# quinlan-lab/STRling

Measured on AMD Instinct MI355X. Metric: reads/sec through extract+cluster, 30x 150 bp WGS; 1/2/4/8 MI355X + CPU ref, higher is better.
Workload: dtype u8/u32 integer; 1 GPU; 1xMI355X: 30x 150 bp PE synthetic WGS, k=2-6 repeat-unit scorer + soft-clip scan + device pair logic + on-GPU radix-sort/segmented clustering (BASELINE.json configs[1]+[2]); reads_per_gpu=33554432, read_len=150, unique_reads_per_gpu=33554432, tiles=1, scored_reads=2843008, soft_items=993737, str_reads_clustered=514295, clusters=322142, bounds=5047, parallelism=records sharded over 1 GPU(s), no data-path collective

## Files before the change

### strling_amd/csrc/device_util.h

```cpp
#pragma once
#include <algorithm>
#include "common.h"

namespace strl {

__device__ __forceinline__ void bloom_set(uint32_t *bloom, uint32_t mask, uint64_t m) {
  const uint32_t b0 = (uint32_t)m & mask, b1 = (uint32_t)(m >> 32) & mask;
  atomicOr(&bloom[b0 >> 5], 1u << (b0 & 31u));
  atomicOr(&bloom[b1 >> 5], 1u << (b1 & 31u));
}
__device__ __forceinline__ bool bloom_test(const uint32_t *bloom, uint32_t mask, uint64_t m) {
  const uint32_t b0 = (uint32_t)m & mask;
  if (!((bloom[b0 >> 5] >> (b0 & 31u)) & 1u)) return false;
  const uint32_t b1 = (uint32_t)(m >> 32) & mask;
  return (bloom[b1 >> 5] >> (b1 & 31u)) & 1u;
}


static __global__ void zero_words_kernel(uint32_t *p, size_t n_words) {
  const size_t n4 = n_words / 4, stride = (size_t)gridDim.x * blockDim.x;
  uint4 *q = reinterpret_cast<uint4 *>(p);
  for (size_t i = (size_t)blockIdx.x * blockDim.x + threadIdx.x; i < n4; i += stride) q[i] = make_uint4(0, 0, 0, 0);
  if (blockIdx.x == 0 && threadIdx.x < (n_words & 3)) p[n4 * 4 + threadIdx.x] = 0;
}
static __global__ void zero_words2_kernel(uint32_t *p, size_t n_words, uint32_t *q, size_t m_words) {
  const size_t stride = (size_t)gridDim.x * blockDim.x, i0 = (size_t)blockIdx.x * blockDim.x + threadIdx.x;
  for (size_t i = i0; i < n_words; i += stride) p[i] = 0;
  for (size_t i = i0; i < m_words; i += stride) q[i] = 0;
}
static inline hipError_t zero_words2(void *p, size_t bytes, void *q, size_t qbytes, hipStream_t st) {
  const size_t w = std::max(bytes, qbytes) / 4;
  if (!w) return hipSuccess;
  const unsigned blocks = (unsigned)std::min<size_t>((w + 255) / 256, 1024);
  hipLaunchKernelGGL(zero_words2_kernel, dim3(blocks), dim3(256), 0, st, static_cast<uint32_t *>(p), bytes / 4, static_cast<uint32_t *>(q), qbytes / 4);
  return hipGetLastError();
}
static inline hipError_t zero_words(void *p, size_t bytes, hipStream_t st) {
  const size_t words = bytes / 4;
  if (!words) return hipSuccess;
  const unsigned blocks = (unsigned)std::min<size_t>((words / 4 + 255) / 256 + 1, 1024);
  hipLaunchKernelGGL(zero_words_kernel, dim3(blocks), dim3(256), 0, st, static_cast<uint32_t *>(p), words);
  return hipGetLastError();
}
}
```

### strling_amd/csrc/pair.hip

```cpp
#include <string.h>
#include <algorithm>
#include "common.h"
#include "device_util.h"
#include "sort.h"
#include "front.h"

namespace strl {

constexpr uint16_t F_PROPER = 0x2, F_REVERSE = 0x10, F_MREVERSE = 0x20, F_SECONDARY = 0x100, F_SUPPL = 0x800;
constexpr int PAIR_MAXM = 15;
constexpr int PAIR_LONG_MAX = PAIR_LONG_MAX_ITEMS;
constexpr uint32_t PAIR_SPILL_CAP = 1u << 16;

struct PairParams {
  uint32_t n;
  uint32_t tail_start;
  const strl_pair_rec *rec;
  const uint64_t *qhash;
  const uint32_t *whole;
  const strl_soft_rec *soft;
  const uint32_t *d_n_soft;
  uint32_t scap;
  uint32_t *bloom;
  uint32_t bloom_mask;
  uint64_t *item_key;
  uint32_t *item_val;
  uint32_t item_cap;
  uint32_t *pc;
  strl_tread *emit;
  uint64_t *emit_key;
  uint32_t *emit_val;
  uint32_t emit_cap;
  double p;
  uint32_t min_mapq;
  int32_t frag_median;
  uint32_t *spill;
  const uint64_t *qref;
  const uint8_t *qarena;
};

__device__ inline bool qname_differs(const PairParams &P, uint32_t r0, uint32_t r1) {
  if (!P.qref) return false;
  const uint64_t a = P.qref[r0], b = P.qref[r1];
  if ((a & 255u) != (b & 255u)) return true;
  const uint8_t *x = P.qarena + (a >> 8), *y = P.qarena + (b >> 8);
  for (uint32_t j = 0; j < (uint32_t)(a & 255u); ++j) if (x[j] != y[j]) return true;
  return false;
}

__global__ __launch_bounds__(1024) void pair_soft_items_kernel(PairParams P) {
  __shared__ uint32_t wcnt[128];
  __shared__ uint32_t base_sh;
  constexpr int U = 2;
  const int lane = threadIdx.x & 63, wave = threadIdx.x >> 6;
  const unsigned long long below = (1ull << lane) - 1ull;
  uint32_t n_src = *P.d_n_soft;
  if (n_src > P.scap) n_src = P.scap;
  for (uint32_t b0 = blockIdx.x * (1024u * U); b0 < n_src; b0 += gridDim.x * (1024u * U)) {
    uint64_t m[U];
    bool hot[U];
    unsigned long long bal[U];
#pragma unroll
    for (int u = 0; u < U; ++u) {
      const uint32_t j = b0 + 1024u * u + threadIdx.x;
      hot[u] = false;
      m[u] = 0;
      if (j < n_src) {
        const strl_soft_rec s = P.soft[j];
        hot[u] = (STRL_RES_COUNT(s.res_first) | STRL_RES_COUNT(s.res_after)) != 0;
        if (hot[u]) {
          m[u] = fmix64(P.qhash[s.read_side >> 1]);
          bloom_set(P.bloom, P.bloom_mask, m[u]);
        }
      }
    }
#pragma unroll
    for (int u = 0; u < U; ++u) {
      bal[u] = __ballot(hot[u]);
      if (lane == 0) wcnt[u * 16 + wave] = (uint32_t)__popcll(bal[u]);
    }
    __syncthreads();
    if (threadIdx.x == 0) {
      uint32_t tot = 0;
      for (int w = 0; w < 16 * U; ++w) { const uint32_t c = wcnt[w]; wcnt[w] = tot; tot += c; }
      base_sh = tot ? atomicAdd(&P.pc[PC_ITEMS], tot) : 0u;
    }
    __syncthreads();
#pragma unroll
    for (int u = 0; u < U; ++u) {
      if (hot[u]) {
        const uint32_t d = base_sh + wcnt[u * 16 + wave] + (uint32_t)__popcll(bal[u] & below);
        if (d < P.item_cap) { P.item_key[d] = m[u]; P.item_val[d] = 0x80000000u | (b0 + 1024u * u + threadIdx.x); }
        else atomicOr(&P.pc[PC_ERR], PAIR_ERR_ITEMS);
      }
    }
    __syncthreads();
  }
}

constexpr int PR_STAGE = 1024, PR_ILP = 8;
__global__ __launch_bounds__(256) void pair_probe_kernel(PairParams P) {
  __shared__ uint32_t stage[4][PR_STAGE + 64 * PR_ILP];
  const int lane = threadIdx.x & 63, wave = threadIdx.x >> 6;
  uint32_t *buf = stage[wave];
  const uint64_t n_waves = (uint64_t)gridDim.x * 4u;
  const uint64_t gw = (uint64_t)blockIdx.x * 4u + wave;
  const uint64_t per = (((P.n + n_waves - 1) / n_waves) + 63ull) & ~63ull;
  const uint64_t r0 = gw * per;
  const uint64_t r1 = r0 + per < P.n ? r0 + per : P.n;
  const unsigned long long below = (1ull << lane) - 1ull;
  uint32_t cnt = 0;
  auto flush = [&]() {
    if (cnt) {
      uint32_t b = 0;
      if (lane == 0) b = atomicAdd(&P.pc[PC_ITEMS], cnt);
      b = __shfl(b, 0);
      __builtin_amdgcn_wave_barrier();
      for (uint32_t i = lane; i < cnt; i += 64) {
        const uint32_t r = buf[i];
        const uint32_t d = b + i;
        if (d < P.item_cap) { P.item_key[d] = fmix64(P.qhash[r]); P.item_val[d] = r; }
        else atomicOr(&P.pc[PC_ERR], PAIR_ERR_ITEMS);
      }
      __builtin_amdgcn_wave_barrier();
      cnt = 0;
    }
  };
  uint64_t cur[PR_ILP], nxt[PR_ILP];
  auto load = [&](uint64_t base, uint64_t (&x)[PR_ILP]) {
#pragma unroll
    for (int j = 0; j < PR_ILP; ++j) {
      const uint64_t r = base + 64ull * j + lane;
      x[j] = r < r1 ? P.qhash[r] : 0ull;
    }
  };
  load(r0, cur);
  for (uint64_t base = r0; base < r1; base += 64 * PR_ILP) {
    load(base + 64 * PR_ILP, nxt);
    uint64_t m[PR_ILP];
    uint32_t w0[PR_ILP];
#pragma unroll
    for (int j = 0; j < PR_ILP; ++j) {
      m[j] = fmix64(cur[j]);
      w0[j] = P.bloom[((uint32_t)m[j] & P.bloom_mask) >> 5];
    }
    bool hit[PR_ILP];
#pragma unroll
    for (int j = 0; j < PR_ILP; ++j) {
      const uint64_t r = base + 64ull * j + lane;
      hit[j] = r < r1 && ((w0[j] >> ((uint32_t)m[j] & 31u)) & 1u);
    }
#pragma unroll
    for (int j = 0; j < PR_ILP; ++j) {
      if (hit[j]) {
        const uint32_t b1 = (uint32_t)(m[j] >> 32) & P.bloom_mask;
        hit[j] = (P.bloom[b1 >> 5] >> (b1 & 31u)) & 1u;
      }
    }
#pragma unroll
    for (int j = 0; j < PR_ILP; ++j) {
      const unsigned long long mk = __ballot(hit[j]);
      if (hit[j]) buf[cnt + __popcll(mk & below)] = (uint32_t)(base + 64ull * j + lane);
      cnt += (uint32_t)__popcll(mk);
    }
    if (cnt >= PR_STAGE) flush();
#pragma unroll
    for (int j = 0; j < PR_ILP; ++j) cur[j] = nxt[j];
  }
  flush();
}

struct DTread {
  int32_t tid;
  uint32_t position;
  uint32_t k, code;
  uint16_t flag;
  uint8_t split, mapq, count, align_length;
  uint32_t qid;
};

__device__ __forceinline__ double p_repeat(const DTread &t) {
  const uint8_t prod = (uint8_t)(t.count * (uint8_t)t.k);
  const uint8_t al = t.align_length ? t.align_length : 1;
  return (double)prod / (double)al;
}
__device__ inline uint32_t min_rev_complement(uint32_t code, uint32_t k) {
  if (k == 0) return code;
  uint32_t c = 0;
  for (int i = (int)k - 1; i >= 0; --i) c = (c << 2) | (3u - ((code >> (2 * (k - 1 - i))) & 3u));
  const uint32_t mask = (1u << (2 * k)) - 1u;
  uint32_t best = c, f = c;
  for (uint32_t j = 0; j < k; ++j) {
    f = ((f << 2) | (f >> (2 * (k - 1)))) & mask;
    best = f < best ? f : best;
  }
  return best;
}
__device__ inline uint32_t canonical_repeat(uint32_t code, uint32_t k) {
  const uint32_t r = min_rev_complement(code, k);
  for (uint32_t j = 0; j < k; ++j) {
    const uint32_t a = (r >> (2 * (k - 1 - j))) & 3u, b = (code >> (2 * (k - 1 - j))) & 3u;
    const uint32_t ra = a ^ 1u, rb = b ^ 1u;
    if (ra != rb) return ra < rb ? r : code;
  }
  return code;
}
__device__ __forceinline__ bool should_reverse(uint16_t f) {
  const bool r = !(f & F_MREVERSE);
  return (f & F_REVERSE) ? !r : r;
}
__device__ inline bool adjust_by(DTread &A, const DTread &B, const PairParams &P, uint32_t B_position) {
  if (A.count == 0) return false;
  const uint32_t half = (uint32_t)((double)A.align_length / 2.0 + 0.5);
  if (B.mapq > P.min_mapq && ((p_repeat(A) > P.p && p_repeat(B) < 0.2) || (!(A.flag & F_PROPER) && A.mapq < P.min_mapq))) {
    if (B.flag & F_REVERSE) {
// ... 152 lines not shown
      mate.code = canonical_repeat(mate.code, mate.k);
      mate.position = 0;
      mate.tid = -1;
      emit(E, self, vidx, seq, *G.err);
      emit(E, mate, vidx, seq, *G.err);
      return;
    }
    const uint32_t mp = mate.position;
    if (adjust_by(mate, self, P, self.position)) emit(E, mate, vidx, seq, *G.err);
    if (adjust_by(self, mate, P, mp)) emit(E, self, vidx, seq, *G.err);
  } else {
    const DTread tr = to_tread(x, *G.err);
    add_soft(G, x, true, tr.k, E, vidx, seq);
    if (stored) stored = false;
    else { S = tr; stored = true; }
  }
}

template <class Ctx> __device__ inline void replay_run(Ctx &G, int m, const EmitStage &E) {
  const PairParams &P = G.P;
  int a = 0;
  while (a < m) {
    int b = a + 1;
    while (b < m && G.item(b).key == G.item(a).key) ++b;
    G.i0 = a; G.i1 = b;
    if (P.qref)
      for (int j = a + 1; j < b; ++j) {
        const PItem &x = G.item(j);
        if (x.val & 0x80000000u) break;
        if (qname_differs(P, G.item(a).val, x.val)) *G.err |= PAIR_ERR_COLLISION;
      }
    bool stored = false;
    DTread S{};
    for (int j = a; j < b; ++j) {
      const PItem &x = G.item(j);
      if (x.val & 0x80000000u) break;
      cache_add(G, x, (uint64_t)x.val, stored, S, E);
    }
    for (int j = a; j < b; ++j) {
      const PItem &x = G.item(j);
      if (x.val & 0x80000000u) break;
      if (x.val >= P.tail_start) cache_add(G, x, (uint64_t)P.n + (uint64_t)(x.val - P.tail_start), stored, S, E);
    }
    a = b;
  }
}


__global__ __launch_bounds__(PG_BLOCK) void pair_groups_kernel(PairParams P) {
  extern __shared__ __attribute__((aligned(16))) uint8_t pg_lds[];
  PItem *items = reinterpret_cast<PItem *>(pg_lds);
  strl_tread *st_t = reinterpret_cast<strl_tread *>(pg_lds + sizeof(PItem) * (PG_BLOCK + PG_HALO));
  uint64_t *st_k = reinterpret_cast<uint64_t *>(st_t + PG_EMIT);
  uint32_t *sh = reinterpret_cast<uint32_t *>(st_k + PG_EMIT);
  uint32_t n_items = P.pc[PC_ITEMS];
  if (n_items > P.item_cap) n_items = P.item_cap;
  const EmitStage E{st_t, st_k, sh, &P};
  for (uint32_t b0 = blockIdx.x * (uint32_t)PG_BLOCK; b0 < n_items; b0 += gridDim.x * (uint32_t)PG_BLOCK) {
    if (threadIdx.x == 0) sh[0] = 0;
    for (uint32_t l = threadIdx.x; l < (uint32_t)(PG_BLOCK + PG_HALO); l += PG_BLOCK) {
      const uint32_t i = b0 + l;
      PItem x{};
      x.key = ~0ull;
      if (i < n_items) {
        x.key = P.item_key[i];
        x.val = P.item_val[i];
        if (x.val & 0x80000000u) {
          const strl_soft_rec s = P.soft[x.val & 0x7fffffffu];
          x.tid = (int32_t)s.read_side; x.pos = (int32_t)s.res_first; x.mtid = (int32_t)s.res_after;
        } else {
          const uint32_t r = x.val;
          const uint4 *rp = reinterpret_cast<const uint4 *>(P.rec + r);
          union { uint4 q[2]; strl_pair_rec o; } u;
          u.q[0] = rp[0];
          u.q[1] = rp[1];
          x.tid = u.o.tid; x.pos = u.o.pos; x.mtid = u.o.mtid; x.mpos = u.o.mpos; x.end = u.o.end;
          x.whole = P.whole[r]; x.flag = u.o.flag; x.clip_l = u.o.clip_l; x.clip_r = u.o.clip_r; x.l_seq = u.o.l_seq;
          x.mapq = u.o.mapq; x.cig = u.o.cig;
        }
      }
      items[l] = x;
    }
    __syncthreads();
    const uint32_t i = b0 + threadIdx.x;
    uint32_t err = 0;
    if (i < n_items) {
      const int me = (int)threadIdx.x;
      const uint32_t lo = (uint32_t)items[me].key;
      const bool head = i == 0 || (me > 0 ? (uint32_t)items[me - 1].key : (uint32_t)P.item_key[i - 1]) != lo;
      if (head) {
        uint64_t perm = 0;
        int m = 0;
        bool too_long = false;
        for (int j = me; j < PG_BLOCK + PG_HALO && b0 + (uint32_t)j < n_items; ++j) {
          if ((uint32_t)items[j].key != lo) break;
          if (m == PAIR_MAXM) { too_long = true; break; }
          const uint64_t k = items[j].key;
          const uint32_t v = items[j].val;
          int q = m;
          while (q > 0) {
            const PItem &o = items[me + (int)((perm >> (4 * (q - 1))) & 15u)];
            if (o.key > k || (o.key == k && o.val > v)) --q; else break;
          }
          const uint64_t lowmask = (1ull << (4 * q)) - 1ull;
          perm = (perm & lowmask) | ((uint64_t)(j - me) << (4 * q)) | ((perm & ~lowmask) << 4);
          ++m;
        }
        if (too_long) {
          const uint32_t sl = atomicAdd(&P.pc[PC_SPILL], 1u);
          if (sl < PAIR_SPILL_CAP) P.spill[sl] = i;
          else err |= PAIR_ERR_RUN;
        } else {
          GroupCtx G{P, items, perm, me, 0, 0, &err, false};
          replay_run(G, m, E);
        }
      }
    }
    if (err) atomicOr(&P.pc[PC_ERR], err);
    __syncthreads();
    uint32_t ne = sh[0];
    if (ne > (uint32_t)PG_EMIT) ne = PG_EMIT;
    if (threadIdx.x == 0) sh[1] = ne ? atomicAdd(&P.pc[PC_EMIT], ne) : 0u;
    __syncthreads();
    const uint32_t base = sh[1];
    for (uint32_t e = threadIdx.x; e < ne; e += PG_BLOCK) {
      const uint32_t d = base + e;
      if (d < P.emit_cap) {
        const uint4 *src = reinterpret_cast<const uint4 *>(st_t + e);
        uint4 *dst = reinterpret_cast<uint4 *>(P.emit + d);
        dst[0] = src[0]; dst[1] = src[1];
        P.emit_key[d] = st_k[e];
        P.emit_val[d] = d;
      } else atomicOr(&P.pc[PC_ERR], PAIR_ERR_EMIT);
    }
    __syncthreads();
  }
}

__global__ __launch_bounds__(PAIR_LONG_MAX) void pair_long_kernel(PairParams P) {
  __shared__ PItem raw[PAIR_LONG_MAX], srt[PAIR_LONG_MAX];
  __shared__ strl_tread st_t[PG_EMIT];
  __shared__ uint64_t st_k[PG_EMIT];
  __shared__ uint32_t sh[4];
  uint32_t n_items = P.pc[PC_ITEMS];
  if (n_items > P.item_cap) n_items = P.item_cap;
  uint32_t n_spill = P.pc[PC_SPILL];
  if (n_spill > PAIR_SPILL_CAP) n_spill = PAIR_SPILL_CAP;
  const EmitStage E{st_t, st_k, sh, &P};
  for (uint32_t e = blockIdx.x; e < n_spill; e += gridDim.x) {
    const uint32_t i0 = P.spill[e];
    const uint32_t lo = (uint32_t)P.item_key[i0];
    if (threadIdx.x == 0) { sh[0] = 0; sh[3] = PAIR_LONG_MAX; }
    __syncthreads();
    const uint32_t i = i0 + threadIdx.x;
    const bool mine = i < n_items && (uint32_t)P.item_key[i] == lo;
    if (!mine) atomicMin(&sh[3], threadIdx.x);
    __syncthreads();
    const uint32_t m = sh[3];
    const bool beyond = m == (uint32_t)PAIR_LONG_MAX && i0 + PAIR_LONG_MAX < n_items && (uint32_t)P.item_key[i0 + PAIR_LONG_MAX] == lo;
    uint32_t err = 0;
    if (beyond) { if (threadIdx.x == 0) atomicOr(&P.pc[PC_ERR], PAIR_ERR_RUN); __syncthreads(); continue; }
    if (threadIdx.x < m) {
      PItem x{};
      x.key = P.item_key[i];
      x.val = P.item_val[i];
      if (x.val & 0x80000000u) {
        const strl_soft_rec s = P.soft[x.val & 0x7fffffffu];
        x.tid = (int32_t)s.read_side; x.pos = (int32_t)s.res_first; x.mtid = (int32_t)s.res_after;
      } else {
        const strl_pair_rec o = P.rec[x.val];
        x.tid = o.tid; x.pos = o.pos; x.mtid = o.mtid; x.mpos = o.mpos; x.end = o.end;
        x.whole = P.whole[x.val]; x.flag = o.flag; x.clip_l = o.clip_l; x.clip_r = o.clip_r; x.l_seq = o.l_seq;
        x.mapq = o.mapq; x.cig = o.cig;
      }
      raw[threadIdx.x] = x;
    }
    __syncthreads();
    if (threadIdx.x < m) {
      const PItem x = raw[threadIdx.x];
      uint32_t rank = 0;
      for (uint32_t j = 0; j < m; ++j) {
        const PItem &o = raw[j];
        if (o.key < x.key || (o.key == x.key && o.val < x.val)) ++rank;
      }
      srt[rank] = x;
    }
    __syncthreads();
    if (threadIdx.x == 0) {
      GroupCtx G{P, srt, 0, 0, 0, 0, &err, true};
      replay_run(G, (int)m, E);
      if (err) atomicOr(&P.pc[PC_ERR], err);
    }
    __syncthreads();
    uint32_t ne = sh[0];
    if (ne > (uint32_t)PG_EMIT) ne = PG_EMIT;
    if (threadIdx.x == 0) sh[1] = ne ? atomicAdd(&P.pc[PC_EMIT], ne) : 0u;
    __syncthreads();
    const uint32_t base = sh[1];
    for (uint32_t k = threadIdx.x; k < ne; k += blockDim.x) {
      const uint32_t d = base + k;
      if (d < P.emit_cap) { P.emit[d] = st_t[k]; P.emit_key[d] = st_k[k]; P.emit_val[d] = d; }
      else atomicOr(&P.pc[PC_ERR], PAIR_ERR_EMIT);
    }
    __syncthreads();
  }
}

__global__ __launch_bounds__(256) void pair_order_kernel(const uint32_t *pc, uint32_t emit_cap, const strl_tread *emit, const uint32_t *perm,
                                                         strl_tread *out, uint32_t *n_out) {
  uint32_t n = pc[PC_EMIT];
  if (n > emit_cap) n = emit_cap;
  const uint32_t i = blockIdx.x * 256u + threadIdx.x;
  if (i == 0) *n_out = n;
  if (i >= n) return;
  const uint4 *src = reinterpret_cast<const uint4 *>(emit + perm[i]);
  uint4 *dst = reinterpret_cast<uint4 *>(out + i);
  dst[0] = src[0];
  dst[1] = src[1];
}

__device__ inline DTread dtread_from(const strl_tread &t) {
  DTread d{};
  d.tid = t.tid; d.position = t.position; d.flag = t.flag; d.split = t.split; d.mapq = t.mapping_quality; d.count = t.repeat_count;
  d.align_length = t.align_length; d.qid = (uint32_t)t.qname_id;
  for (int j = 0; j < 6 && t.repeat[j]; ++j) {
    uint32_t c = 1;
    switch (t.repeat[j]) { case 'C': c = 0; break; case 'A': c = 1; break; case 'T': c = 2; break; case 'G': c = 3; break; }
    d.code = (d.code << 2) | c;
    ++d.k;
  }
  return d;
}
__device__ inline void dtread_to(const DTread &d, strl_tread &t) {
  t.tid = d.tid; t.position = d.position; t.flag = d.flag; t.split = d.split; t.mapping_quality = d.mapq; t.repeat_count = d.count;
  t.align_length = d.align_length;
  for (int j = 0; j < 6; ++j) t.repeat[j] = (uint32_t)j < d.k ? "CATG"[(d.code >> (2 * (d.k - 1 - j))) & 3u] : (char)0;
}
__global__ void pair_rules_kernel(int op, strl_tread *A, const strl_tread *B, PairParams P, uint32_t B_position, int *res) {
  DTread a = dtread_from(*A);
  const DTread b = dtread_from(*B);
  if (op == 0) *res = adjust_by(a, b, P, B_position) ? 1 : 0;
  else if (op == 1) *res = unplaced_pair(a, b, P) ? 1 : 0;
  else { a.code = canonical_repeat(a.code, a.k); *res = 0; }
  dtread_to(a, *A);
}

}

using namespace strl;

extern "C" int strl_pair_rule_device(strl_ctx *c, int op, strl_tread *A, const strl_tread *B, const strl_opts *o, uint32_t B_position, int *result) {
  if (!c || !A || !B || !o || !result || op < 0 || op > 2) { set_error("bad argument"); return STRL_ERR_ARG; }
  STRL_HIP(hipSetDevice(c->device));
  DevBuf buf;
  int rc;
  if ((rc = buf.reserve(2 * sizeof(strl_tread) + 16))) return rc;
  strl_tread *dA = buf.as<strl_tread>(), *dB = dA + 1;
  int *dres = reinterpret_cast<int *>(dB + 1);
  STRL_HIP(hipMemcpyAsync(dA, A, sizeof *A, hipMemcpyHostToDevice, c->stream));
  STRL_HIP(hipMemcpyAsync(dB, B, sizeof *B, hipMemcpyHostToDevice, c->stream));
  PairParams P{};
  P.p = o->proportion_repeat; P.min_mapq = o->min_mapq; P.frag_median = o->median_fragment_length;
  hipLaunchKernelGGL(pair_rules_kernel, dim3(1), dim3(1), 0, c->stream, op, dA, dB, P, B_position, dres);
  STRL_HIP(hipGetLastError());
  STRL_HIP(hipMemcpyAsync(A, dA, sizeof *A, hipMemcpyDeviceToHost, c->stream));
  STRL_HIP(hipMemcpyAsync(result, dres, sizeof(int), hipMemcpyDeviceToHost, c->stream));
  STRL_HIP(hipStreamSynchronize(c->stream));
  buf.release();
  return STRL_OK;
}

int strl_pair_order(strl_ctx *c, hipStream_t on_stream) {
  const bool on_main = !on_stream || on_stream == c->stream;
  if (on_main) { const int rcj = side_join(c); if (rcj) return rcj; }
  if (!c->n_treads_dev) { set_error("no strl_extract_device call on this context"); return STRL_ERR_ARG; }
  if (c->pair_ordered) return STRL_OK;
  hipStream_t st = on_main ? c->stream : on_stream;
  const uint32_t ecap = c->tread_cap;
  uint64_t *ok = nullptr;
  uint32_t *ov = nullptr;
  const int e = radix_sort_pairs(st, c->pair_cnt.as<uint32_t>() + PC_EMIT, ecap, c->po_key, c->po_val, c->po_key_alt, c->po_val_alt, c->sort_scratch.p,
                                 c->sort_scratch.cap, 0, c->po_bits, &ok, &ov);
  if (e) { set_error("radix_sort_pairs failed: %s", hipGetErrorString((hipError_t)e)); return STRL_ERR_HIP; }
  uint32_t *n_out = reinterpret_cast<uint32_t *>(c->treads.as<uint8_t>() + (size_t)ecap * sizeof(strl_tread));
  hipLaunchKernelGGL(pair_order_kernel, dim3((ecap + 255) / 256), dim3(256), 0, st, c->pair_cnt.as<uint32_t>(), ecap, c->p_emit.as<strl_tread>(), ov,
                     c->treads.as<strl_tread>(), n_out);
  STRL_HIP(hipGetLastError());
  c->n_treads_dev = n_out;
  c->pair_ordered = true;
  return STRL_OK;
}

int strl_pair_device(strl_ctx *c, uint64_t n, const strl_pair_soa *pp, const uint32_t *whole, const strl_soft_rec *soft,
                     const uint32_t *d_n_soft, uint64_t soft_cap, int64_t n_tail, uint64_t item_cap, uint64_t tread_cap, hipStream_t on_stream) {
  if (n > strl_record_limit()) { set_error("pair logic: more than %llu records in one device pass", (unsigned long long)strl_record_limit()); return STRL_ERR_LIMIT; }
  if (n_tail < 0 || (uint64_t)n_tail > n) { set_error("strl_pair_device: n_tail must be in [0, n]"); return STRL_ERR_ARG; }
  if (item_cap > 0x7ffffff0ull || tread_cap > 0x7ffffff0ull) { set_error("pair capacities too large"); return STRL_ERR_ARG; }
  hipStream_t st = on_stream ? on_stream : c->stream;
  int rc;
  if (st == c->stream && (rc = side_join(c))) return rc;
  c->pair_on_side = false;
  const uint32_t icap = (uint32_t)std::max<uint64_t>(item_cap, 1024), ecap = (uint32_t)std::max<uint64_t>(tread_cap, 1024);
  int ebits = 3;
  while (ebits < 40 && ((2 * n) >> (ebits - 2))) ++ebits;
  const size_t sb = std::max(radix_sort_scratch_bytes(icap, 32), radix_sort_scratch_bytes(ecap, ebits));
  if ((rc = c->p_key0.reserve((size_t)std::max(icap, ecap) * 8)) || (rc = c->p_key1.reserve((size_t)std::max(icap, ecap) * 8)) ||
      (rc = c->p_val0.reserve((size_t)std::max(icap, ecap) * 4)) || (rc = c->p_val1.reserve((size_t)std::max(icap, ecap) * 4)) ||
      (rc = c->p_emit.reserve((size_t)ecap * sizeof(strl_tread))) || (rc = c->treads.reserve((size_t)ecap * sizeof(strl_tread) + 64)) ||
      (rc = c->sort_scratch.reserve(sb)) || (rc = c->pair_cnt.reserve(PC_WORDS * 4 + 64)) || (rc = c->p_spill.reserve((size_t)PAIR_SPILL_CAP * 4)))
    return rc;
  void *jt = nullptr;
  size_t jt_bytes = 0;
  radix_sort_tables(c->sort_scratch.p, icap, 32, &jt, &jt_bytes);
  STRL_HIP(zero_words2(c->pair_cnt.p, PC_WORDS * 4 + 64, jt, jt_bytes, st));
  PairParams P{};
  P.n = (uint32_t)n;
  P.tail_start = (uint32_t)(n - (uint64_t)n_tail);
  P.rec = pp->rec; P.qhash = pp->qhash;
  P.whole = whole; P.soft = soft; P.d_n_soft = d_n_soft;
  P.scap = (uint32_t)std::max<uint64_t>(std::min<uint64_t>(soft_cap, 2 * n), 1);
  P.bloom = c->bloom.as<uint32_t>(); P.bloom_mask = c->bloom_mask;
  P.item_key = c->p_key0.as<uint64_t>(); P.item_val = c->p_val0.as<uint32_t>(); P.item_cap = icap;
  P.pc = c->pair_cnt.as<uint32_t>();
  P.emit = c->p_emit.as<strl_tread>(); P.emit_key = c->p_key0.as<uint64_t>(); P.emit_val = c->p_val0.as<uint32_t>(); P.emit_cap = ecap;
  P.p = c->opts.proportion_repeat; P.min_mapq = c->opts.min_mapq; P.frag_median = c->opts.median_fragment_length;
  P.spill = c->p_spill.as<uint32_t>();
  const bool names = c->x_front && c->front && pp->rec == c->x_rows.as<strl_pair_rec>();
  P.qref = names ? c->front->qref.as<uint64_t>() : nullptr;
  P.qarena = names ? c->front->qarena.as<uint8_t>() : nullptr;
  hipEvent_t *ev = c->timing ? c->pev : nullptr;
  if (ev) STRL_HIP(hipEventRecord(ev[0], st));
  if (n) {
    hipLaunchKernelGGL(pair_soft_items_kernel, dim3(512), dim3(1024), 0, st, P);
    if (ev) STRL_HIP(hipEventRecord(ev[1], st));
    static const int env_p = getenv("STRL_GRID_P") ? atoi(getenv("STRL_GRID_P")) : 0;
    const int pblocks = (int)std::min<uint64_t>((n + 2047) / 2048, env_p > 0 ? (uint64_t)env_p : 1024);
    hipLaunchKernelGGL(pair_probe_kernel, dim3(pblocks), dim3(256), 0, st, P);
    STRL_HIP(hipGetLastError());
  }
  else if (ev) STRL_HIP(hipEventRecord(ev[1], st));
  if (ev) STRL_HIP(hipEventRecord(ev[2], st));
  uint64_t *ik = nullptr;
  uint32_t *iv = nullptr;
  int e = radix_sort_pairs(st, P.pc + PC_ITEMS, icap, c->p_key0.as<uint64_t>(), c->p_val0.as<uint32_t>(), c->p_key1.as<uint64_t>(),
                           c->p_val1.as<uint32_t>(), c->sort_scratch.p, c->sort_scratch.cap, 0, 32, &ik, &iv, true);
  if (e) { set_error("radix_sort_pairs failed: %s", hipGetErrorString((hipError_t)e)); return STRL_ERR_HIP; }
  if (ev) STRL_HIP(hipEventRecord(ev[3], st));
  P.item_key = ik; P.item_val = iv;
  const bool in0 = ik == c->p_key0.as<uint64_t>();
  uint64_t *ek = in0 ? c->p_key1.as<uint64_t>() : c->p_key0.as<uint64_t>();
  uint32_t *evl = in0 ? c->p_val1.as<uint32_t>() : c->p_val0.as<uint32_t>();
  P.emit_key = ek; P.emit_val = evl;
  if (n) {
    const size_t pg_shmem = sizeof(PItem) * (PG_BLOCK + PG_HALO) + (sizeof(strl_tread) + 8) * PG_EMIT + 16;
    if (!c->pg_attr_done) {
      STRL_HIP(hipFuncSetAttribute(reinterpret_cast<const void *>(pair_groups_kernel), hipFuncAttributeMaxDynamicSharedMemorySize, (int)pg_shmem));
      c->pg_attr_done = true;
    }
    hipLaunchKernelGGL(pair_groups_kernel, dim3((unsigned)std::min<uint32_t>((icap + PG_BLOCK - 1) / PG_BLOCK, 8192)), dim3(PG_BLOCK), pg_shmem, st, P);
    STRL_HIP(hipGetLastError());
    hipLaunchKernelGGL(pair_long_kernel, dim3(64), dim3(PAIR_LONG_MAX), 0, st, P);
    STRL_HIP(hipGetLastError());
  }
  if (ev) STRL_HIP(hipEventRecord(ev[4], st));
  c->po_key = ek; c->po_val = evl; c->po_key_alt = ik; c->po_val_alt = iv; c->po_bits = ebits;
  c->pair_ordered = false;
  c->n_treads_dev = c->pair_cnt.as<uint32_t>() + PC_EMIT;
  if (ev) STRL_HIP(hipEventRecord(ev[5], st));
  c->tread_cap = ecap;
  c->pair_item_cap = icap;
  return STRL_OK;
}
```

### strling_amd/csrc/score.hip

```cpp
#include <stdarg.h>
#include <string.h>
#include <sys/mman.h>
#include <algorithm>
#include <atomic>
#include <chrono>
#include <mutex>
#include <thread>
#include <vector>
#include "common.h"
#include "host_score.h"
#include "front.h"
#include "device_util.h"
#include "score_core.h"
#include "score_tables.h"
#include "sort.h"

namespace strl {

static thread_local char g_err[512] = "";
void set_error(const char *fmt, ...) {
  va_list ap;
  va_start(ap, fmt);
  vsnprintf(g_err, sizeof g_err, fmt, ap);
  va_end(ap);
// ... 1637 lines not shown
  if ((rc = c->x_rows.grow((size_t)(at + n) * sizeof(strl_pair_rec), (size_t)at * sizeof(strl_pair_rec), c->stream)) ||
      (rc = c->x_qhash.grow((size_t)(at + n) * 8, (size_t)at * 8, c->stream)) || (rc = c->x_whole.grow((size_t)(at + n) * 4, (size_t)at * 4, c->stream)))
    return rc;
  strl_read_soa d = *s;
  const hipMemcpyKind kind = s->mem == STRL_MEM_DEVICE ? hipMemcpyDeviceToDevice : hipMemcpyHostToDevice;
  if (s->mem != STRL_MEM_DEVICE && (rc = stage_batch(c, s, nullptr, &d, nullptr))) return rc;
  STRL_HIP(hipMemcpyAsync(c->x_rows.as<strl_pair_rec>() + at, pp->rec, (size_t)n * sizeof(strl_pair_rec), kind, c->stream));
  STRL_HIP(hipMemcpyAsync(c->x_qhash.as<uint64_t>() + at, pp->qhash, (size_t)n * 8, kind, c->stream));
  return extract_add_scored(c, &d, at);
}

int strl_extract_finish(strl_ctx *c, int64_t n_tail, uint64_t item_cap, uint64_t tread_cap) {
  if (!c) { set_error("null argument"); return STRL_ERR_ARG; }
  if (!c->x_open && !c->x_mode) { set_error("strl_extract_finish without strl_extract_begin"); return STRL_ERR_ARG; }
  STRL_HIP(hipSetDevice(c->device));
  const uint64_t n = c->x_n;
  if (n_tail < 0 || (uint64_t)n_tail > n) { set_error("strl_extract_finish: n_tail must be in [0, n]"); return STRL_ERR_ARG; }
  if (!item_cap) item_cap = n / 8 + 65536;
  if (!tread_cap) tread_cap = n / 16 + 65536;
  item_cap = std::min<uint64_t>(item_cap, 3 * n + 16);
  tread_cap = std::min<uint64_t>(tread_cap, 8 * n + 16);
  c->x_open = false; c->x_mode = true;
  c->ex_n = n; c->ex_soft_cap = c->x_soft_cap;
  const strl_pair_soa dp{c->x_rows.as<strl_pair_rec>(), c->x_qhash.as<uint64_t>()};
  return strl_pair_device(c, n, &dp, c->x_whole.as<uint32_t>(), c->x_soft.as<strl_soft_rec>(), c->x_cnt.as<uint32_t>() + XC_SOFT,
                          std::max<uint64_t>(c->x_soft_cap, 1), n_tail, item_cap, tread_cap);
}

int strl_treads_fetch(strl_ctx *c, strl_tread *out, uint64_t cap, uint64_t *n_out, strl_score_stats *stats) {
  if (!c) { set_error("null argument"); return STRL_ERR_ARG; }
  if (!c->n_treads_dev) { set_error("strl_treads_fetch: no strl_extract_device call on this context"); return STRL_ERR_ARG; }
  STRL_HIP(hipSetDevice(c->device));
  { const int rc0 = strl_pair_order(c); if (rc0) return rc0; }
  uint32_t raw[CNT_WORDS], pc[PC_WORDS], xc[XC_WORDS];
  STRL_HIP(hipMemcpyAsync(raw, c->counters.p, CNT_WORDS * 4, hipMemcpyDeviceToHost, c->stream));
  STRL_HIP(hipMemcpyAsync(pc, c->pair_cnt.p, PC_WORDS * 4, hipMemcpyDeviceToHost, c->stream));
  if (c->x_mode) STRL_HIP(hipMemcpyAsync(xc, c->x_cnt.p, XC_WORDS * 4, hipMemcpyDeviceToHost, c->stream));
  STRL_HIP(hipStreamSynchronize(c->stream));
  if (c->x_mode) {
    raw[CNT_SKIP] = xc[XC_SKIP]; raw[CNT_QUEUE] = xc[XC_QUEUE]; raw[CNT_SBW] = xc[XC_SBW]; raw[CNT_SBS] = xc[XC_SBS]; raw[CNT_SOFT] = xc[XC_SOFT];
  }
  if (stats) {
    memset(stats, 0, sizeof *stats);
    stats->n_reads = c->ex_n; stats->n_skipped = raw[CNT_SKIP]; stats->n_scored = raw[CNT_QUEUE]; stats->n_soft_items = raw[CNT_SOFT];
    stats->n_stage_b_whole = raw[CNT_SBW]; stats->n_stage_b_soft = raw[CNT_SBS];
  }
  if (n_out) *n_out = pc[PC_EMIT];
  if (c->x_mode && xc[XC_OVERFLOW]) { set_error("chunked extract: soft-clip records of a chunk were dropped (%u kept of %u)", xc[XC_SOFT], xc[XC_SOFT_ITEMS]); return STRL_ERR_CAPACITY; }
  if (raw[CNT_SOFT] > c->ex_soft_cap) { set_error("soft-clip queue overflow: %u items, capacity %llu (raise item_cap)", raw[CNT_SOFT], (unsigned long long)c->ex_soft_cap); return STRL_ERR_CAPACITY; }
  const uint32_t err = pc[PC_ERR];
  if (err & PAIR_ERR_ITEMS) { set_error("pair logic: %u join items, capacity %u (raise item_cap)", pc[PC_ITEMS], c->pair_item_cap); return STRL_ERR_CAPACITY; }
  if (err & PAIR_ERR_EMIT) { set_error("pair logic: %u treads, capacity %u (raise tread_cap)", pc[PC_EMIT], c->tread_cap); return STRL_ERR_CAPACITY; }
  if (err & PAIR_ERR_COLLISION) { set_error("pair logic: two different qnames share one 64-bit hash (use the host pair logic, strl_pair_reads: it keys on the string)"); return STRL_ERR_FORMAT; }
  if (err & (PAIR_ERR_RUN | PAIR_ERR_LOCAL)) { set_error("pair logic: more than %d join items share the low 32 bits of their qname hash (use the host pair logic, strl_pair_reads)", strl::PAIR_LONG_MAX_ITEMS); return STRL_ERR_FORMAT; }
  if (err & PAIR_ERR_ASSERT) { set_error("repeat_count >= 256 (doAssert extract.nim:72)"); return STRL_ERR_ASSERT; }
  const uint64_t n = pc[PC_EMIT];
  if (out) {
    if (n > cap) { set_error("tread capacity %llu too small, need %llu", (unsigned long long)cap, (unsigned long long)n); return STRL_ERR_CAPACITY; }
    if (n) STRL_HIP(hipMemcpy(out, c->treads.p, (size_t)n * sizeof(strl_tread), hipMemcpyDeviceToHost));
  }
  return STRL_OK;
}

int strl_ctx_pair_times(strl_ctx *c, double ms[5]) {
  if (!c || !ms) return STRL_ERR_ARG;
  STRL_HIP(hipSetDevice(c->device));
  STRL_HIP(hipStreamSynchronize(c->stream));
  for (int k = 0; k < 5; ++k) {
    float f = 0.f;
    if (c->timing) (void)hipEventElapsedTime(&f, c->pev[k], c->pev[k + 1]);
    ms[k] = f;
  }
  return STRL_OK;
}


static int front_fill_done(strl_ctx *c, strl::FrontSlot &S, strl_front_chunk *done) {
  STRL_HIP(hipEventSynchronize(S.ev_b));
  S.b_pending = false;
  const strl::FrontInfo &I = S.h_info[1];
  if (I.err & strl::FRONT_ERR_LSEQ) { set_error("a record's l_seq is outside [0, %d]", STRL_MAX_READ_LEN); return STRL_ERR_ARG; }
  if (done) {
    done->n_records = I.n_records; done->n_primary = I.n_primary; done->last_placed = I.last_placed; done->tail_primary = I.tail_primary;
    done->max_l_seq = I.max_l_seq; done->scan_slow_segments = I.slow_segments;
  }
  return STRL_OK;
}

static int front_adopt_big(strl_ctx *c, strl::strl_front *F, uint64_t at) {
  strl::FrontBigAlloc *B = F->big;
  if (!B) return STRL_OK;
  if (B->th.joinable()) B->th.join();
  F->big = nullptr;
  if (B->rc) {
    set_error("%s", B->err.c_str());
    const int rc = B->rc;
    for (strl::DevBuf *b : {&B->rows, &B->qhash, &B->whole, &B->qref, &B->fragw, &B->qarena}) b->release();
    delete B;
    return rc;
  }
  struct Mv { strl::DevBuf *cur, *big; size_t used; };
  const Mv mv[6] = {{&c->x_rows, &B->rows, (size_t)at * sizeof(strl_pair_rec)}, {&c->x_qhash, &B->qhash, (size_t)at * 8}, {&c->x_whole, &B->whole, (size_t)at * 4},
                    {&F->qref, &B->qref, (size_t)at * 8}, {&F->fragw, &B->fragw, (size_t)at * 4}, {&F->qarena, &B->qarena, (size_t)F->qarena_used}};
  for (const Mv &m : mv) {
    if (m.big->cap <= m.cur->cap) { m.big->release(); continue; }
    if (m.used) STRL_HIP(hipMemcpyAsync(m.big->p, m.cur->p, std::min(m.used, m.cur->cap), hipMemcpyDeviceToDevice, c->stream));
    F->trash.push_back(*m.cur);
// ... 474 lines not shown
```

Baseline: 29.16 billion reads/s.

## Add optional bucket-count join path for pair logic, stage hashes in LDS

New measurement: 29.26 billion reads/s, median of 6. Within noise of the previous version (+0.4%).

```diff
diff --git a/strling_amd/csrc/device_util.h b/strling_amd/csrc/device_util.h
--- a/strling_amd/csrc/device_util.h
+++ b/strling_amd/csrc/device_util.h
@@ -26,11 +26,17 @@
 static __global__ void zero_words2_kernel(uint32_t *p, size_t n_words, uint32_t *q, size_t m_words) {
   const size_t stride = (size_t)gridDim.x * blockDim.x, i0 = (size_t)blockIdx.x * blockDim.x + threadIdx.x;
   for (size_t i = i0; i < n_words; i += stride) p[i] = 0;
-  for (size_t i = i0; i < m_words; i += stride) q[i] = 0;
+  if ((reinterpret_cast<uintptr_t>(q) & 15) == 0) {
+    uint4 *q4 = reinterpret_cast<uint4 *>(q);
+    const size_t m4 = m_words / 4;
+    for (size_t i = i0; i < m4; i += stride) q4[i] = make_uint4(0, 0, 0, 0);
+    for (size_t i = m4 * 4 + i0; i < m_words; i += stride) q[i] = 0;
+  } else
+    for (size_t i = i0; i < m_words; i += stride) q[i] = 0;
 }
 static inline hipError_t zero_words2(void *p, size_t bytes, void *q, size_t qbytes, hipStream_t st) {
-  const size_t w = std::max(bytes, qbytes) / 4;
-  if (!w) return hipSuccess;
+  if (bytes < 4 && qbytes < 4) return hipSuccess;
+  const size_t w = std::max(bytes, qbytes / 4) / 4 + 1;
   const unsigned blocks = (unsigned)std::min<size_t>((w + 255) / 256, 1024);
   hipLaunchKernelGGL(zero_words2_kernel, dim3(blocks), dim3(256), 0, st, static_cast<uint32_t *>(p), bytes / 4, static_cast<uint32_t *>(q), qbytes / 4);
   return hipGetLastError();
diff --git a/strling_amd/csrc/pair.hip b/strling_amd/csrc/pair.hip
--- a/strling_amd/csrc/pair.hip
+++ b/strling_amd/csrc/pair.hip
@@ -37,7 +37,13 @@
   uint32_t *spill;
   const uint64_t *qref;
   const uint8_t *qarena;
+  uint32_t *bcnt;
+  uint32_t bmask;
 };
+
+__device__ __forceinline__ void bucket_count(const PairParams &P, uint64_t m) {
+  if (P.bcnt) (void)__hip_atomic_fetch_add(&P.bcnt[(uint32_t)m & P.bmask], 1u, __ATOMIC_RELAXED, __HIP_MEMORY_SCOPE_AGENT);
+}
 
 __device__ inline bool qname_differs(const PairParams &P, uint32_t r0, uint32_t r1) {
   if (!P.qref) return false;
@@ -90,7 +96,7 @@
     for (int u = 0; u < U; ++u) {
       if (hot[u]) {
         const uint32_t d = base_sh + wcnt[u * 16 + wave] + (uint32_t)__popcll(bal[u] & below);
-        if (d < P.item_cap) { P.item_key[d] = m[u]; P.item_val[d] = 0x80000000u | (b0 + 1024u * u + threadIdx.x); }
+        if (d < P.item_cap) { P.item_key[d] = m[u]; P.item_val[d] = 0x80000000u | (b0 + 1024u * u + threadIdx.x); bucket_count(P, m[u]); }
         else atomicOr(&P.pc[PC_ERR], PAIR_ERR_ITEMS);
       }
     }
@@ -98,11 +104,14 @@
   }
 }
 
-constexpr int PR_STAGE = 1024, PR_ILP = 8;
+constexpr int PR_STAGE = 320, PR_ILP = 8;
+static_assert(4 * (PR_STAGE + 64 * PR_ILP) * 12 <= 40 * 1024, "pair_probe_kernel: four blocks per CU");
 __global__ __launch_bounds__(256) void pair_probe_kernel(PairParams P) {
+  __shared__ uint64_t stage_m[4][PR_STAGE + 64 * PR_ILP];
   __shared__ uint32_t stage[4][PR_STAGE + 64 * PR_ILP];
   const int lane = threadIdx.x & 63, wave = threadIdx.x >> 6;
   uint32_t *buf = stage[wave];
+  uint64_t *bufm = stage_m[wave];
   const uint64_t n_waves = (uint64_t)gridDim.x * 4u;
   const uint64_t gw = (uint64_t)blockIdx.x * 4u + wave;
   const uint64_t per = (((P.n + n_waves - 1) / n_waves) + 63ull) & ~63ull;
@@ -117,9 +126,8 @@
       b = __shfl(b, 0);
       __builtin_amdgcn_wave_barrier();
       for (uint32_t i = lane; i < cnt; i += 64) {
-        const uint32_t r = buf[i];
         const uint32_t d = b + i;
-        if (d < P.item_cap) { P.item_key[d] = fmix64(P.qhash[r]); P.item_val[d] = r; }
+        if (d < P.item_cap) { const uint64_t m = bufm[i]; P.item_key[d] = m; P.item_val[d] = buf[i]; bucket_count(P, m); }
         else atomicOr(&P.pc[PC_ERR], PAIR_ERR_ITEMS);
       }
       __builtin_amdgcn_wave_barrier();
@@ -160,7 +168,7 @@
 #pragma unroll
     for (int j = 0; j < PR_ILP; ++j) {
       const unsigned long long mk = __ballot(hit[j]);
-      if (hit[j]) buf[cnt + __popcll(mk & below)] = (uint32_t)(base + 64ull * j + lane);
+      if (hit[j]) { const uint32_t q = cnt + (uint32_t)__popcll(mk & below); buf[q] = (uint32_t)(base + 64ull * j + lane); bufm[q] = m[j]; }
       cnt += (uint32_t)__popcll(mk);
     }
     if (cnt >= PR_STAGE) flush();
@@ -419,12 +427,15 @@
   PItem *items = reinterpret_cast<PItem *>(pg_lds);
   strl_tread *st_t = reinterpret_cast<strl_tread *>(pg_lds + sizeof(PItem) * (PG_BLOCK + PG_HALO));
   uint64_t *st_k = reinterpret_cast<uint64_t *>(st_t + PG_EMIT);
-  uint32_t *sh = reinterpret_cast<uint32_t *>(st_k + PG_EMIT);
+  uint64_t *jperm = st_k + PG_EMIT;
+  uint32_t *sh = reinterpret_cast<uint32_t *>(jperm + PG_BLOCK);
+  uint16_t *jdesc = reinterpret_cast<uint16_t *>(sh + 4);
   uint32_t n_items = P.pc[PC_ITEMS];
   if (n_items > P.item_cap) n_items = P.item_cap;
   const EmitStage E{st_t, st_k, sh, &P};
   for (uint32_t b0 = blockIdx.x * (uint32_t)PG_BLOCK; b0 < n_items; b0 += gridDim.x * (uint32_t)PG_BLOCK) {
     if (threadIdx.x == 0) sh[0] = 0;
+    jdesc[threadIdx.x] = 0;
     for (uint32_t l = threadIdx.x; l < (uint32_t)(PG_BLOCK + PG_HALO); l += PG_BLOCK) {
       const uint32_t i = b0 + l;
       PItem x{};
@@ -453,14 +464,14 @@
     uint32_t err = 0;
     if (i < n_items) {
       const int me = (int)threadIdx.x;
-      const uint32_t lo = (uint32_t)items[me].key;
-      const bool head = i == 0 || (me > 0 ? (uint32_t)items[me - 1].key : (uint32_t)P.item_key[i - 1]) != lo;
+      const uint32_t lo = (uint32_t)items[me].key & P.bmask;
+      const bool head = i == 0 || ((me > 0 ? (uint32_t)items[me - 1].key : (uint32_t)P.item_key[i - 1]) & P.bmask) != lo;
       if (head) {
         uint64_t perm = 0;
         int m = 0;
         bool too_long = false;
         for (int j = me; j < PG_BLOCK + PG_HALO && b0 + (uint32_t)j < n_items; ++j) {
-          if ((uint32_t)items[j].key != lo) break;
+          if (((uint32_t)items[j].key & P.bmask) != lo) break;
           if (m == PAIR_MAXM) { too_long = true; break; }
           const uint64_t k = items[j].key;
           const uint32_t v = items[j].val;
@@ -478,9 +489,27 @@
           if (sl < PAIR_SPILL_CAP) P.spill[sl] = i;
           else err |= PAIR_ERR_RUN;
         } else {
-          GroupCtx G{P, items, perm, me, 0, 0, &err, false};
-          replay_run(G, m, E);
+          int a = 0;
+          for (int g = 0; a < m; ++g) {
+            const uint64_t k = items[me + (int)((perm >> (4 * a)) & 15u)].key;
+            int b = a + 1;
+            while (b < m && items[me + (int)((perm >> (4 * b)) & 15u)].key == k) ++b;
+            if (me + g < PG_BLOCK) { jperm[me + g] = perm >> (4 * a); jdesc[me + g] = (uint16_t)((me << 4) | (b - a)); }
+            else {
+              GroupCtx G{P, items, perm >> (4 * a), me, 0, 0, &err, false};
+              replay_run(G, b - a, E);
+            }
+            a = b;
+          }
         }
+      }
+    }
+    __syncthreads();
+    {
+      const uint32_t jd = jdesc[threadIdx.x];
+      if (jd & 15u) {
+        GroupCtx G{P, items, jperm[threadIdx.x], (int)(jd >> 4), 0, 0, &err, false};
+        replay_run(G, (int)(jd & 15u), E);
       }
     }
     if (err) atomicOr(&P.pc[PC_ERR], err);
@@ -516,15 +545,15 @@
   const EmitStage E{st_t, st_k, sh, &P};
   for (uint32_t e = blockIdx.x; e < n_spill; e += gridDim.x) {
     const uint32_t i0 = P.spill[e];
-    const uint32_t lo = (uint32_t)P.item_key[i0];
+    const uint32_t lo = (uint32_t)P.item_key[i0] & P.bmask;
     if (threadIdx.x == 0) { sh[0] = 0; sh[3] = PAIR_LONG_MAX; }
     __syncthreads();
     const uint32_t i = i0 + threadIdx.x;
-    const bool mine = i < n_items && (uint32_t)P.item_key[i] == lo;
+    const bool mine = i < n_items && ((uint32_t)P.item_key[i] & P.bmask) == lo;
     if (!mine) atomicMin(&sh[3], threadIdx.x);
     __syncthreads();
     const uint32_t m = sh[3];
-    const bool beyond = m == (uint32_t)PAIR_LONG_MAX && i0 + PAIR_LONG_MAX < n_items && (uint32_t)P.item_key[i0 + PAIR_LONG_MAX] == lo;
+    const bool beyond = m == (uint32_t)PAIR_LONG_MAX && i0 + PAIR_LONG_MAX < n_items && ((uint32_t)P.item_key[i0 + PAIR_LONG_MAX] & P.bmask) == lo;
     uint32_t err = 0;
     if (beyond) { if (threadIdx.x == 0) atomicOr(&P.pc[PC_ERR], PAIR_ERR_RUN); __syncthreads(); continue; }
     if (threadIdx.x < m) {
@@ -572,6 +601,114 @@
     __syncthreads();
   }
 }
+
+constexpr uint32_t PB_TILE = 4096;
+constexpr int PAIR_BUCKET_BITS_MIN = 16;
+constexpr int PAIR_BUCKET_BITS_MAX = 22;
+constexpr uint32_t PB_MAX_TILES = (1u << PAIR_BUCKET_BITS_MAX) / PB_TILE;
+constexpr bool PAIR_JOIN_DEFAULT_BUCKET = false;
+
+__device__ __forceinline__ uint32_t pb_excl_scan256(uint32_t v, uint32_t *wsum , uint32_t *total) {
+  const int lane = threadIdx.x & 63, wave = threadIdx.x >> 6;
+  uint32_t inc = v;
+#pragma unroll
+  for (int d = 1; d < 64; d <<= 1) {
+    const uint32_t o = __shfl_up(inc, d);
+    if (lane >= d) inc += o;
+  }
+  if (lane == 63) wsum[wave] = inc;
+  __syncthreads();
+  uint32_t base = 0;
+  for (int w = 0; w < wave; ++w) base += wsum[w];
+  if (total) *total = wsum[0] + wsum[1] + wsum[2] + wsum[3];
+  __syncthreads();
+  return base + inc - v;
+}
+
+__global__ __launch_bounds__(256) void pair_bucket_scan_kernel(uint32_t *cnt, uint32_t *totals) {
+  __shared__ uint32_t wsum[4];
+  uint4 *row = reinterpret_cast<uint4 *>(cnt + (size_t)blockIdx.x * PB_TILE) + threadIdx.x * 4u;
+  uint4 v[4];
+#pragma unroll
+  for (int k = 0; k < 4; ++k) v[k] = row[k];
+  uint32_t sum = 0;
+#pragma unroll
+  for (int k = 0; k < 4; ++k) {
+    const uint32_t a = v[k].x, b = v[k].y, c = v[k].z, d = v[k].w;
+    v[k].x = sum; v[k].y = sum + a; v[k].z = sum + a + b; v[k].w = sum + a + b + c;
+    sum += a + b + c + d;
+  }
+  uint32_t total;
+  const uint32_t base = pb_excl_scan256(sum, wsum, &total);
+#pragma unroll
+  for (int k = 0; k < 4; ++k) { v[k].x += base; v[k].y += base; v[k].z += base; v[k].w += base; row[k] = v[k]; }
+  if (threadIdx.x == 0) totals[blockIdx.x] = total;
+}
+
+constexpr int PB_ILP = 4;
+__global__ __launch_bounds__(256) void pair_bucket_scatter_kernel(PairParams P, uint64_t *kout, uint32_t *vout, const uint32_t *totals, uint32_t n_tiles) {
+  __shared__ uint32_t tbase[PB_MAX_TILES];
+  __shared__ uint32_t wsum[4];
+  uint32_t n_items = P.pc[PC_ITEMS];
+  if (n_items > P.item_cap) n_items = P.item_cap;
+  if ((uint64_t)blockIdx.x * (256u * PB_ILP) >= n_items) return;
+  {
+    const uint32_t per = (n_tiles + 255u) / 256u, t0 = threadIdx.x * per;
+    uint32_t sum = 0;
+    for (uint32_t k = t0; k < t0 + per && k < n_tiles; ++k) sum += totals[k];
+    uint32_t run = pb_excl_scan256(sum, wsum, nullptr);
+    for (uint32_t k = t0; k < t0 + per && k < n_tiles; ++k) { tbase[k] = run; run += totals[k]; }
+  }
+  __syncthreads();
+  uint32_t err = 0;
+  for (uint64_t i0 = (uint64_t)blockIdx.x * (256u * PB_ILP); i0 < n_items; i0 += (uint64_t)gridDim.x * (256u * PB_ILP)) {
+    uint64_t key[PB_ILP];
+    uint32_t val[PB_ILP], slot[PB_ILP];
+    bool in[PB_ILP];
+#pragma unroll
+    for (int u = 0; u < PB_ILP; ++u) {
+      const uint64_t i = i0 + 256u * u + threadIdx.x;
+      in[u] = i < n_items;
+      key[u] = in[u] ? P.item_key[i] : 0ull;
+      val[u] = in[u] ? P.item_val[i] : 0u;
+    }
+#pragma unroll
+    for (int u = 0; u < PB_ILP; ++u) {
+      const uint32_t b = (uint32_t)key[u] & P.bmask;
+      slot[u] = in[u] ? tbase[b / PB_TILE] + atomicAdd(&P.bcnt[b], 1u) : 0u;
+    }
+#pragma unroll
+    for (int u = 0; u < PB_ILP; ++u) {
+      if (!in[u]) continue;
+      if (slot[u] < n_items) { kout[slot[u]] = key[u]; vout[slot[u]] = val[u]; }
+      else err |= PAIR_ERR_LOCAL;
+    }
+  }
+  if (err) atomicOr(&P.pc[PC_ERR], err);
+}
+
+struct JoinPlan { bool bucket; int bits; };
+static int join_plan(uint32_t icap, JoinPlan *j) {
+  int b = PAIR_BUCKET_BITS_MIN;
+  while (b < 31 && 1.25 * (double)(1u << b) < (double)icap) ++b;
+  j->bucket = PAIR_JOIN_DEFAULT_BUCKET && b <= PAIR_BUCKET_BITS_MAX;
+  j->bits = std::min(b, PAIR_BUCKET_BITS_MAX);
+  const char *e = getenv("STRL_PAIR_JOIN");
+  if (e && *e) {
+    if (!strcmp(e, "sort")) j->bucket = false;
+    else if (!strcmp(e, "bucket")) j->bucket = true;
+    else { set_error("STRL_PAIR_JOIN must be `sort` or `bucket`, not `%s`", e); return STRL_ERR_ARG; }
+  }
+  e = getenv("STRL_PAIR_BUCKET_BITS");
+  if (e && *e) {
+    const int v = atoi(e);
+    if (v < 1 || v > PAIR_BUCKET_BITS_MAX) { set_error("STRL_PAIR_BUCKET_BITS must be in [1, %d]", PAIR_BUCKET_BITS_MAX); return STRL_ERR_ARG; }
+    j->bits = v;
+  }
+  return STRL_OK;
+}
+static inline uint32_t bucket_table_words(int bits) { return std::max<uint32_t>(1u << bits, PB_TILE); }
+static inline size_t bucket_scratch_bytes(int bits) { const size_t w = bucket_table_words(bits); return 256 + w * 4 + (w / PB_TILE) * 4; }
 
 __global__ __launch_bounds__(256) void pair_order_kernel(const uint32_t *pc, uint32_t emit_cap, const strl_tread *emit, const uint32_t *perm,
                                                          strl_tread *out, uint32_t *n_out) {
@@ -670,7 +807,9 @@
   const uint32_t icap = (uint32_t)std::max<uint64_t>(item_cap, 1024), ecap = (uint32_t)std::max<uint64_t>(tread_cap, 1024);
   int ebits = 3;
   while (ebits < 40 && ((2 * n) >> (ebits - 2))) ++ebits;
-  const size_t sb = std::max(radix_sort_scratch_bytes(icap, 32), radix_sort_scratch_bytes(ecap, ebits));
+  JoinPlan join;
+  if ((rc = join_plan(icap, &join))) return rc;
+  const size_t sb = std::max({radix_sort_scratch_bytes(icap, 32), radix_sort_scratch_bytes(ecap, ebits), bucket_scratch_bytes(PAIR_BUCKET_BITS_MAX)});
   if ((rc = c->p_key0.reserve((size_t)std::max(icap, ecap) * 8)) || (rc = c->p_key1.reserve((size_t)std::max(icap, ecap) * 8)) ||
       (rc = c->p_val0.reserve((size_t)std::max(icap, ecap) * 4)) || (rc = c->p_val1.reserve((size_t)std::max(icap, ecap) * 4)) ||
       (rc = c->p_emit.reserve((size_t)ecap * sizeof(strl_tread))) || (rc = c->treads.reserve((size_t)ecap * sizeof(strl_tread) + 64)) ||
@@ -678,7 +817,13 @@
     return rc;
   void *jt = nullptr;
   size_t jt_bytes = 0;
-  radix_sort_tables(c->sort_scratch.p, icap, 32, &jt, &jt_bytes);
+  uint32_t *btotals = nullptr;
+  const uint32_t btiles = bucket_table_words(join.bits) / PB_TILE;
+  if (join.bucket) {
+    jt = reinterpret_cast<void *>((reinterpret_cast<uintptr_t>(c->sort_scratch.p) + 255) & ~(uintptr_t)255);
+    jt_bytes = (size_t)bucket_table_words(join.bits) * 4;
+    btotals = static_cast<uint32_t *>(jt) + bucket_table_words(join.bits);
+  } else radix_sort_tables(c->sort_scratch.p, icap, 32, &jt, &jt_bytes);
   STRL_HIP(zero_words2(c->pair_cnt.p, PC_WORDS * 4 + 64, jt, jt_bytes, st));
   PairParams P{};
   P.n = (uint32_t)n;
@@ -695,6 +840,8 @@
   const bool names = c->x_front && c->front && pp->rec == c->x_rows.as<strl_pair_rec>();
   P.qref = names ? c->front->qref.as<uint64_t>() : nullptr;
   P.qarena = names ? c->front->qarena.as<uint8_t>() : nullptr;
+  P.bcnt = join.bucket ? static_cast<uint32_t *>(jt) : nullptr;
+  P.bmask = join.bucket ? (1u << join.bits) - 1u : 0xffffffffu;
   hipEvent_t *ev = c->timing ? c->pev : nullptr;
   if (ev) STRL_HIP(hipEventRecord(ev[0], st));
   if (n) {
@@ -707,11 +854,21 @@
   }
   else if (ev) STRL_HIP(hipEventRecord(ev[1], st));
   if (ev) STRL_HIP(hipEventRecord(ev[2], st));
-  uint64_t *ik = nullptr;
-  uint32_t *iv = nullptr;
-  int e = radix_sort_pairs(st, P.pc + PC_ITEMS, icap, c->p_key0.as<uint64_t>(), c->p_val0.as<uint32_t>(), c->p_key1.as<uint64_t>(),
-                           c->p_val1.as<uint32_t>(), c->sort_scratch.p, c->sort_scratch.cap, 0, 32, &ik, &iv, true);
-  if (e) { set_error("radix_sort_pairs failed: %s", hipGetErrorString((hipError_t)e)); return STRL_ERR_HIP; }
+  uint64_t *ik = c->p_key0.as<uint64_t>();
+  uint32_t *iv = c->p_val0.as<uint32_t>();
+  if (join.bucket) {
+    if (n) {
+      ik = c->p_key1.as<uint64_t>(); iv = c->p_val1.as<uint32_t>();
+      hipLaunchKernelGGL(pair_bucket_scan_kernel, dim3(btiles), dim3(256), 0, st, P.bcnt, btotals);
+      const unsigned sblocks = (unsigned)std::min<uint32_t>((icap + 256 * PB_ILP - 1) / (256 * PB_ILP), 2048);
+      hipLaunchKernelGGL(pair_bucket_scatter_kernel, dim3(sblocks), dim3(256), 0, st, P, ik, iv, btotals, btiles);
+      STRL_HIP(hipGetLastError());
+    }
+  } else {
+    const int e = radix_sort_pairs(st, P.pc + PC_ITEMS, icap, c->p_key0.as<uint64_t>(), c->p_val0.as<uint32_t>(), c->p_key1.as<uint64_t>(),
+                                   c->p_val1.as<uint32_t>(), c->sort_scratch.p, c->sort_scratch.cap, 0, 32, &ik, &iv, true);
+    if (e) { set_error("radix_sort_pairs failed: %s", hipGetErrorString((hipError_t)e)); return STRL_ERR_HIP; }
+  }
   if (ev) STRL_HIP(hipEventRecord(ev[3], st));
   P.item_key = ik; P.item_val = iv;
   const bool in0 = ik == c->p_key0.as<uint64_t>();
@@ -719,7 +876,8 @@
   uint32_t *evl = in0 ? c->p_val1.as<uint32_t>() : c->p_val0.as<uint32_t>();
   P.emit_key = ek; P.emit_val = evl;
   if (n) {
-    const size_t pg_shmem = sizeof(PItem) * (PG_BLOCK + PG_HALO) + (sizeof(strl_tread) + 8) * PG_EMIT + 16;
+    const size_t pg_shmem = sizeof(PItem) * (PG_BLOCK + PG_HALO) + (sizeof(strl_tread) + 8) * PG_EMIT + (8 + 2) * PG_BLOCK + 16;
+    static_assert(sizeof(PItem) * (PG_BLOCK + PG_HALO) + (sizeof(strl_tread) + 8) * PG_EMIT + (8 + 2) * PG_BLOCK + 16 <= 40 * 1024, "pair_groups_kernel: four blocks per CU");
     if (!c->pg_attr_done) {
       STRL_HIP(hipFuncSetAttribute(reinterpret_cast<const void *>(pair_groups_kernel), hipFuncAttributeMaxDynamicSharedMemorySize, (int)pg_shmem));
       c->pg_attr_done = true;
diff --git a/strling_amd/csrc/score.hip b/strling_amd/csrc/score.hip
--- a/strling_amd/csrc/score.hip
+++ b/strling_amd/csrc/score.hip
@@ -1713,7 +1713,7 @@
   if (err & PAIR_ERR_ITEMS) { set_error("pair logic: %u join items, capacity %u (raise item_cap)", pc[PC_ITEMS], c->pair_item_cap); return STRL_ERR_CAPACITY; }
   if (err & PAIR_ERR_EMIT) { set_error("pair logic: %u treads, capacity %u (raise tread_cap)", pc[PC_EMIT], c->tread_cap); return STRL_ERR_CAPACITY; }
   if (err & PAIR_ERR_COLLISION) { set_error("pair logic: two different qnames share one 64-bit hash (use the host pair logic, strl_pair_reads: it keys on the string)"); return STRL_ERR_FORMAT; }
-  if (err & (PAIR_ERR_RUN | PAIR_ERR_LOCAL)) { set_error("pair logic: more than %d join items share the low 32 bits of their qname hash (use the host pair logic, strl_pair_reads)", strl::PAIR_LONG_MAX_ITEMS); return STRL_ERR_FORMAT; }
+  if (err & (PAIR_ERR_RUN | PAIR_ERR_LOCAL)) { set_error("pair logic: more than %d join items share one bucket of the qname-hash join (use the host pair logic, strl_pair_reads)", strl::PAIR_LONG_MAX_ITEMS); return STRL_ERR_FORMAT; }
   if (err & PAIR_ERR_ASSERT) { set_error("repeat_count >= 256 (doAssert extract.nim:72)"); return STRL_ERR_ASSERT; }
   const uint64_t n = pc[PC_EMIT];
   if (out) {
```
